# MIT-REALM/gcbf-pytorch

Hardware: NVIDIA H100
Metric: agent*steps/sec (train step, device-timed) (higher is better)
Workload: dtype f32 via 3xfp16 tensor-core products (fp32 accumulate)

## Files before the change

gcbf-pytorch_b200/csrc/gemm_wgmma_f16.cu:

```cuda
#include <cuda.h>
#include <cuda_fp16.h>
#include <stdlib.h>

#include "common.cuh"
#include "sm90_ptx.cuh"

namespace gcbf {
namespace th {

using namespace ptx;

constexpr int BM = 128;
constexpr int BK = 32;
constexpr int SUB_N = 128;
constexpr int WG_K = 16;
constexpr int NUM_THREADS = 384;
constexpr int EPI_THREADS = 256;
constexpr int KCH_MAX = 256 / BK;
constexpr int MN_BOX = 64;
constexpr int STAGES = 4;
constexpr int A_BYTES = BM * BK * 2;
constexpr int B_BYTES = SUB_N * BK * 2;
constexpr int STAGE_BYTES = 2 * A_BYTES + 2 * B_BYTES;
constexpr int PARK_PITCH = SUB_N + 8;
constexpr int PARK_BYTES = BM * PARK_PITCH * 4;
static_assert(PARK_BYTES <= STAGES * STAGE_BYTES, "the second half of a 256-wide tile is parked in the stage ring");
constexpr int SMEM_BYTES = STAGES * STAGE_BYTES + PARK_BYTES + 1024  + 256 ;

enum { EPI_FWD = 0, EPI_DGRAD = 1, EPI_WGRAD = 2 };

struct EpiParams {
  int mode;
  const float* alpha;
  const float* bias;
  int act;
  const float* relu_src;
  int ld_relu;
  const __half* relu_hi;
  int ld_relu_h;
  int accumulate;
  size_t split_stride;
  const uint32_t* amax_a; int a_sr, a_sc;
  const uint32_t* amax_b; int b_sr, b_sc;
  uint32_t* amax_out;
  __half* out_h;
  int ld_out_h;
  uint32_t* out_tile_amax;
  int out_amax_stride;
  float* colsum;
};

__host__ __device__ __forceinline__ uint32_t scale_bits_from_amax(uint32_t amax_bits) {
  const int e = (int)((amax_bits >> 23) & 0xffu);
  if (e == 0 || e == 255) return 0x3f800000u;
  int se = 127 + 14 - (e - 127);
  se = se < 2 ? 2 : (se > 252 ? 252 : se);
  return (uint32_t)se << 23;
}
__host__ __device__ __forceinline__ uint32_t inv_pow2_bits(uint32_t s_bits) { return (uint32_t)(254 - (int)(s_bits >> 23)) << 23; }

template <bool MN_MAJOR>
__device__ __forceinline__ uint64_t tile_desc(uint32_t tile_addr, int kk) {
  if (MN_MAJOR) {
    return make_smem_desc(tile_addr + (uint32_t)(kk * WG_K * 128), BK * 128, 1024, 128);
  }
  return make_smem_desc(tile_addr + (uint32_t)(kk * WG_K * 2), 16, 8 * BK * 2, BK * 2);
}

template <bool MN_MAJOR>
__device__ __forceinline__ void load_tile(uint8_t* dst, const CUtensorMap* map, uint64_t* bar, int mn0, int k0, int rows) {
  if (MN_MAJOR) {
    for (int j = 0; j < rows / MN_BOX; ++j) tma_load_2d(dst + j * (BK * 128), map, bar, mn0 + j * MN_BOX, k0);
  } else {
    tma_load_2d(dst, map, bar, k0, mn0);
  }
}

__device__ __forceinline__ void epi_sync() { asm volatile("bar.sync 1, %0;" ::"n"(EPI_THREADS) : "memory"); }

template <int BN, bool A_MN, bool B_MN>
__global__ void __launch_bounds__(NUM_THREADS, 1)
gemm_h_kernel(const __grid_constant__ CUtensorMap map_a_hi, const __grid_constant__ CUtensorMap map_a_lo,
              const __grid_constant__ CUtensorMap map_b_hi, const __grid_constant__ CUtensorMap map_b_lo,
              float* __restrict__ C, int ldc, int Mo, int No, int tiles_n, int kblocks_per_split, int kblocks_total, int KCH, EpiParams ep) {
  constexpr int NSUB = BN / SUB_N;
  constexpr int MODE = A_MN ? EPI_WGRAD : (B_MN ? EPI_DGRAD : EPI_FWD);
  extern __shared__ uint8_t smem_raw[];
  uint8_t* smem = reinterpret_cast<uint8_t*>((reinterpret_cast<uintptr_t>(smem_raw) + 1023) & ~uintptr_t(1023));
  float* park0 = reinterpret_cast<float*>(smem + STAGES * STAGE_BYTES);
  float* park1 = reinterpret_cast<float*>(smem);
  uint64_t* bars = reinterpret_cast<uint64_t*>(smem + STAGES * STAGE_BYTES + PARK_BYTES);
  uint64_t* full = bars;
  uint64_t* empty = bars + STAGES;
  uint32_t* red = reinterpret_cast<uint32_t*>(bars + 2 * STAGES);

  const int warp = threadIdx.x >> 5, lane = threadIdx.x & 31;
  const int kb0 = blockIdx.y * kblocks_per_split;
  const int kb1 = min(kblocks_total, kb0 + kblocks_per_split);
  const int nkb = kb1 - kb0;
  const int m0 = (blockIdx.x / tiles_n) * BM, n0t = (blockIdx.x % tiles_n) * BN;

  if (threadIdx.x == 0) {
    tma_prefetch_desc(&map_a_hi);
    tma_prefetch_desc(&map_a_lo);
    tma_prefetch_desc(&map_b_hi);
    tma_prefetch_desc(&map_b_lo);
    for (int s = 0; s < STAGES; ++s) { mbar_init(&full[s], 1); mbar_init(&empty[s], 2); }
    fence_barrier_init();
  }
  __syncthreads();

  if (warp < 4) {
    if (threadIdx.x == 0) {
      int stage = 0;
      uint32_t phase = 0;
      for (int sub = 0; sub < NSUB; ++sub) {
        for (int kb = kb0; kb < kb1; ++kb) {
          mbar_wait(&empty[stage], phase ^ 1);
          uint8_t* st = smem + stage * STAGE_BYTES;
          mbar_expect_tx(&full[stage], STAGE_BYTES);
          load_tile<A_MN>(st, &map_a_hi, &full[stage], m0, kb * BK, BM);
          load_tile<A_MN>(st + A_BYTES, &map_a_lo, &full[stage], m0, kb * BK, BM);
          load_tile<B_MN>(st + 2 * A_BYTES, &map_b_hi, &full[stage], n0t + sub * SUB_N, kb * BK, SUB_N);
          load_tile<B_MN>(st + 2 * A_BYTES + B_BYTES, &map_b_lo, &full[stage], n0t + sub * SUB_N, kb * BK, SUB_N);
          if (++stage == STAGES) { stage = 0; phase ^= 1; }
        }
      }
    }
  } else {
    if (nkb > 0) {
      const int tid = threadIdx.x - 128;
      const int wg = tid >> 7;
      const int wl = (tid >> 5) & 3;
      const uint32_t a_off = (uint32_t)wg * 4096u;
      int stage = 0;
      uint32_t phase = 0;
      for (int sub = 0; sub < NSUB; ++sub) {
        const int n0 = n0t + sub * SUB_N;
        float acc[64];
#pragma unroll
        for (int j = 0; j < 64; ++j) acc[j] = 0.f;
        for (int kc = 0; kc < nkb; kc += KCH) {
          const int kstart = (kb0 + kc) * BK;
          const int ia = A_MN ? (kstart >> 7) * ep.a_sr + (m0 >> 8) * ep.a_sc : (m0 >> 7) * ep.a_sr + (kstart >> 8) * ep.a_sc;
          const int ib = B_MN ? (kstart >> 7) * ep.b_sr + (n0 >> 8) * ep.b_sc : 0;
          const float cs = __uint_as_float(inv_pow2_bits(scale_bits_from_amax(__ldg(ep.amax_a + ia)))) *
                           __uint_as_float(inv_pow2_bits(scale_bits_from_amax(__ldg(ep.amax_b + ib))));
          float d[64];
#pragma unroll
          for (int j = 0; j < 64; ++j) d[j] = 0.f;
          const int kend = min(nkb, kc + KCH);
          for (int kb = kc; kb < kend; ++kb) {
            mbar_wait(&full[stage], phase);
            const uint32_t st = smem_u32(smem + stage * STAGE_BYTES);
            const uint32_t a_hi = st + a_off, a_lo = st + A_BYTES + a_off, b_hi = st + 2 * A_BYTES, b_lo = st + 2 * A_BYTES + B_BYTES;
#pragma unroll
            for (int j = 0; j < 64; ++j) fence_operand(d[j]);
            wgmma_fence();
#pragma unroll
            for (int kk = 0; kk < BK / WG_K; ++kk) {
              const uint64_t dah = tile_desc<A_MN>(a_hi, kk), dal = tile_desc<A_MN>(a_lo, kk);
              const uint64_t dbh = tile_desc<B_MN>(b_hi, kk), dbl = tile_desc<B_MN>(b_lo, kk);
              wgmma_m64n128k16_f16<A_MN ? 1 : 0, B_MN ? 1 : 0>(d, dal, dbh, (kb > kc || kk > 0) ? 1u : 0u);
              wgmma_m64n128k16_f16<A_MN ? 1 : 0, B_MN ? 1 : 0>(d, dah, dbl, 1u);
              wgmma_m64n128k16_f16<A_MN ? 1 : 0, B_MN ? 1 : 0>(d, dah, dbh, 1u);
            }
            wgmma_commit();
            wgmma_wait_all();
#pragma unroll
            for (int j = 0; j < 64; ++j) fence_operand(d[j]);
            if ((tid & 127) == 0) mbar_arrive(&empty[stage]);
            if (++stage == STAGES) { stage = 0; phase ^= 1; }
          }
#pragma unroll
          for (int j = 0; j < 64; ++j) acc[j] = __fmaf_rn(d[j], cs, acc[j]);
        }
        if (sub == 1) epi_sync();
        float* park = sub ? park1 : park0;
        const int r0 = wg * 64 + wl * 16 + (lane >> 2);
#pragma unroll
        for (int j = 0; j < 64; j += 4) {
          const int c = 8 * (j >> 2) + 2 * (lane & 3);
          *reinterpret_cast<float2*>(park + r0 * PARK_PITCH + c) = make_float2(acc[j], acc[j + 1]);
          *reinterpret_cast<float2*>(park + (r0 + 8) * PARK_PITCH + c) = make_float2(acc[j + 2], acc[j + 3]);
        }
      }
      epi_sync();

      constexpr int CG4 = BN / 4;
      constexpr int ROWS_PER_ITER = EPI_THREADS / CG4;
      const int cg = tid % CG4;
      const int c = cg * 4;
      const int col = n0t + c;
      float* const pk = (c < SUB_N ? park0 : park1) + (c & (SUB_N - 1));
      const float alpha = ep.alpha ? __ldg(ep.alpha) : 1.f;
      float bias4[4] = {0.f, 0.f, 0.f, 0.f};
      if (MODE == EPI_FWD && ep.bias) {
        const float inv_alpha = 1.f / alpha;
#pragma unroll
        for (int u = 0; u < 4; ++u) bias4[u] = (col + u < No) ? __ldg(ep.bias + col + u) * inv_alpha : 0.f;
      }
      float tmax = 0.f;
      for (int r = tid / CG4; r < BM; r += ROWS_PER_ITER) {
        const int row = m0 + r;
        float4* p = reinterpret_cast<float4*>(pk + r * PARK_PITCH);
        float v[4];
        const float4 s = *p;
        v[0] = s.x; v[1] = s.y; v[2] = s.z; v[3] = s.w;
#pragma unroll
        for (int u = 0; u < 4; ++u) {
          float y = (v[u] + bias4[u]) * alpha;
          if (MODE == EPI_FWD) {
            if (ep.act == GCBF_ACT_RELU) y = fmaxf(y, 0.f);
            else if (ep.act == GCBF_ACT_TANH) y = tanhf(y);
          }
          const bool ok = row < Mo && col + u < No;
          if (MODE == EPI_DGRAD && ok) {
            if (ep.relu_src) y = (__ldg(ep.relu_src + (size_t)row * ep.ld_relu + col + u) > 0.f) ? y : 0.f;
            else if (ep.relu_hi) y = (__half2float(ep.relu_hi[(size_t)row * ep.ld_relu_h + col + u]) > 0.f) ? y : 0.f;
          }
          v[u] = ok ? y : 0.f;
          tmax = fmaxf(tmax, fabsf(v[u]));
        }
        *p = make_float4(v[0], v[1], v[2], v[3]);
      }
      float s_tile = 1.f;
      if (MODE != EPI_WGRAD && ep.out_h) {
        const uint32_t wmax = __reduce_max_sync(0xffffffffu, __float_as_uint(tmax));
        if (lane == 0) red[tid >> 5] = wmax;
        epi_sync();
        uint32_t m = 0;
#pragma unroll
        for (int w = 0; w < EPI_THREADS / 32; ++w) m = max(m, red[w]);
        s_tile = __uint_as_float(scale_bits_from_amax(m));
        if (tid == 0 && m0 < Mo && n0t < No) ep.out_tile_amax[(size_t)(m0 >> 7) * ep.out_amax_stride + (n0t >> 8)] = m;
      }
      float out_max = 0.f;
      const bool vec_c = C && (ldc & 3) == 0 && (reinterpret_cast<uintptr_t>(C) & 15) == 0;
      const size_t plane = (size_t)Mo * ep.ld_out_h;
      for (int r = tid / CG4; r < BM; r += ROWS_PER_ITER) {
        const int row = m0 + r;
        if (row >= Mo || col >= No) continue;
        const float4 s = *reinterpret_cast<const float4*>(pk + r * PARK_PITCH);
        const float v[4] = {s.x, s.y, s.z, s.w};
        const int nv = min(4, No - col);
        if (C) {
          float* dst = C + (size_t)blockIdx.y * ep.split_stride + (size_t)row * ldc + col;
          if (ep.accumulate) {
#pragma unroll
            for (int u = 0; u < 4; ++u)
              if (u < nv) { const float o = v[u] + dst[u]; dst[u] = o; out_max = fmaxf(out_max, fabsf(o)); }
          } else if (vec_c && nv == 4) {
            *reinterpret_cast<float4*>(dst) = s;
          } else {
#pragma unroll
            for (int u = 0; u < 4; ++u)
              if (u < nv) dst[u] = v[u];
          }
        }
        if (MODE != EPI_WGRAD && ep.out_h) {
          const float y0 = v[0] * s_tile, y1 = v[1] * s_tile, y2 = v[2] * s_tile, y3 = v[3] * s_tile;
          const __half2 h01 = __floats2half2_rn(y0, y1), h23 = __floats2half2_rn(y2, y3);
          const float2 f01 = __half22float2(h01), f23 = __half22float2(h23);
          const __half2 l01 = __floats2half2_rn(__fsub_rn(y0, f01.x), __fsub_rn(y1, f01.y));
          const __half2 l23 = __floats2half2_rn(__fsub_rn(y2, f23.x), __fsub_rn(y3, f23.y));
          __half* dh = ep.out_h + (size_t)row * ep.ld_out_h + col;
          if (nv == 4) {
            *reinterpret_cast<uint2*>(dh) = make_uint2(*reinterpret_cast<const uint32_t*>(&h01), *reinterpret_cast<const uint32_t*>(&h23));
            *reinterpret_cast<uint2*>(dh + plane) = make_uint2(*reinterpret_cast<const uint32_t*>(&l01), *reinterpret_cast<const uint32_t*>(&l23));
          } else {
            const __half hs[4] = {__low2half(h01), __high2half(h01), __low2half(h23), __high2half(h23)};
            const __half ls[4] = {__low2half(l01), __high2half(l01), __low2half(l23), __high2half(l23)};
            for (int u = 0; u < nv; ++u) { dh[u] = hs[u]; dh[plane + u] = ls[u]; }
          }
        }
      }
      if (ep.amax_out && !ep.accumulate) out_max = fmaxf(out_max, tmax);
      if (MODE == EPI_DGRAD && ep.colsum) epi_sync();
      if (MODE == EPI_DGRAD && ep.colsum && tid < BN) {
        const float* pc = (tid < SUB_N ? park0 : park1) + (tid & (SUB_N - 1));
        float csum = 0.f;
#pragma unroll 8
        for (int r = 0; r < BM; ++r) csum += pc[r * PARK_PITCH];
        if (n0t + tid < No) ep.colsum[(size_t)(blockIdx.x / tiles_n) * No + n0t + tid] = csum;
      }
      if (ep.amax_out) {
        const uint32_t m = __reduce_max_sync(0xffffffffu, __float_as_uint(out_max));
        if (lane == 0 && m) atomicMax(ep.amax_out, m);
      }
    }
  }
}
__global__ void amax_kernel(const float* __restrict__ src, int ld, int rows, int cols, uint32_t* __restrict__ slot, int vec4) {
  float m = 0.f;
  if (vec4) {
    const int w = cols >> 2;
    for (int r = blockIdx.x; r < rows; r += gridDim.x) {
      const float4* p = reinterpret_cast<const float4*>(src + (size_t)r * ld);
      for (int c = threadIdx.x; c < w; c += blockDim.x) {
        const float4 x = __ldg(p + c);
        m = fmaxf(fmaxf(m, fmaxf(fabsf(x.x), fabsf(x.y))), fmaxf(fabsf(x.z), fabsf(x.w)));
      }
    }
  } else {
    for (int r = blockIdx.x; r < rows; r += gridDim.x)
      for (int c = threadIdx.x; c < cols; c += blockDim.x) m = fmaxf(m, fabsf(__ldg(src + (size_t)r * ld + c)));
  }
  const uint32_t w = __reduce_max_sync(0xffffffffu, __float_as_uint(m));
  __shared__ uint32_t part[32];
  if ((threadIdx.x & 31) == 0) part[threadIdx.x >> 5] = w;
  __syncthreads();
  if (threadIdx.x < 32) {
    uint32_t v = threadIdx.x < (blockDim.x >> 5) ? part[threadIdx.x] : 0u;
    v = __reduce_max_sync(0xffffffffu, v);
    if (threadIdx.x == 0 && v) atomicMax(slot, v);
  }
}

constexpr int SPLIT_ROWS = 64;
__global__ void split_h_kernel(const float* __restrict__ src, int ld, int rows, int cols, const uint32_t* __restrict__ amax,
                               __half* __restrict__ dst, int ld_h, float* __restrict__ colsum) {
  const float s = __uint_as_float(scale_bits_from_amax(__ldg(amax)));
  const int c = (blockIdx.x * 32 + threadIdx.x) * 2;
  const int r0 = blockIdx.y * SPLIT_ROWS;
  const size_t plane = (size_t)rows * ld_h;
  float s0 = 0.f, s1 = 0.f;
  if (c < cols) {
    const bool pair = (c + 1 < cols);
    const int r1 = min(rows, r0 + SPLIT_ROWS);
    for (int r = r0 + threadIdx.y; r < r1; r += blockDim.y) {
      const float* p = src + (size_t)r * ld + c;
      const float x0 = __ldg(p), x1 = pair ? __ldg(p + 1) : 0.f;
      const float y0 = x0 * s, y1 = x1 * s;
      const __half2 hi = __floats2half2_rn(y0, y1);
      const float2 hf = __half22float2(hi);
      const __half2 lo = __floats2half2_rn(__fsub_rn(y0, hf.x), __fsub_rn(y1, hf.y));
      __half* d = dst + (size_t)r * ld_h + c;
      if (pair) {
        *reinterpret_cast<__half2*>(d) = hi;
        *reinterpret_cast<__half2*>(d + plane) = lo;
      } else {
        d[0] = __low2half(hi);
        d[plane] = __low2half(lo);
      }
      s0 += x0; s1 += x1;
    }
  }
  if (colsum) {
    __shared__ float red[8][64];
    red[threadIdx.y][2 * threadIdx.x] = s0;
    red[threadIdx.y][2 * threadIdx.x + 1] = s1;
    __syncthreads();
    if (threadIdx.y == 0) {
      float t0 = 0.f, t1 = 0.f;
#pragma unroll
      for (int y = 0; y < 8; ++y) { t0 += red[y][2 * threadIdx.x]; t1 += red[y][2 * threadIdx.x + 1]; }
      if (c < cols) colsum[(size_t)blockIdx.y * cols + c] = t0;
      if (c + 1 < cols) colsum[(size_t)blockIdx.y * cols + c + 1] = t1;
    }
  }
}

__device__ __forceinline__ void split4(const float4 x, float s, uint2& hi, uint2& lo) {
  const float y0 = x.x * s, y1 = x.y * s, y2 = x.z * s, y3 = x.w * s;
  const __half2 h01 = __floats2half2_rn(y0, y1), h23 = __floats2half2_rn(y2, y3);
  const float2 f01 = __half22float2(h01), f23 = __half22float2(h23);
  const __half2 l01 = __floats2half2_rn(__fsub_rn(y0, f01.x), __fsub_rn(y1, f01.y));
  const __half2 l23 = __floats2half2_rn(__fsub_rn(y2, f23.x), __fsub_rn(y3, f23.y));
  hi.x = *reinterpret_cast<const uint32_t*>(&h01); hi.y = *reinterpret_cast<const uint32_t*>(&h23);
  lo.x = *reinterpret_cast<const uint32_t*>(&l01); lo.y = *reinterpret_cast<const uint32_t*>(&l23);
}

__global__ void __launch_bounds__(256) split_h4_kernel(const float* __restrict__ src, int ld, int rows, int cols,
                                                       const uint32_t* __restrict__ amax, __half* __restrict__ dst, int ld_h,
                                                       float* __restrict__ colsum) {
  const float s = __uint_as_float(scale_bits_from_amax(__ldg(amax)));
  const int c = (blockIdx.x * 32 + threadIdx.x) * 4;
  const int r0 = blockIdx.y * SPLIT_ROWS;
  const size_t plane = (size_t)rows * ld_h;
  float cs[4] = {0.f, 0.f, 0.f, 0.f};
  if (c < cols) {
    const int r1 = min(rows, r0 + SPLIT_ROWS);
    for (int r = r0 + threadIdx.y; r < r1; r += 32) {
      float4 x[4];
#pragma unroll
      for (int u = 0; u < 4; ++u)
        x[u] = (r + 8 * u < r1) ? __ldg(reinterpret_cast<const float4*>(src + (size_t)(r + 8 * u) * ld + c)) : make_float4(0.f, 0.f, 0.f, 0.f);
#pragma unroll
      for (int u = 0; u < 4; ++u) {
        if (r + 8 * u < r1) {
          uint2 hi, lo;
          split4(x[u], s, hi, lo);
          __half* d = dst + (size_t)(r + 8 * u) * ld_h + c;
          *reinterpret_cast<uint2*>(d) = hi;
          *reinterpret_cast<uint2*>(d + plane) = lo;
          cs[0] += x[u].x; cs[1] += x[u].y; cs[2] += x[u].z; cs[3] += x[u].w;
        }
      }
    }
  }
  if (colsum) {
    __shared__ float red[8][128];
#pragma unroll
    for (int j = 0; j < 4; ++j) red[threadIdx.y][4 * threadIdx.x + j] = cs[j];
    __syncthreads();
    if (threadIdx.y < 4) {
      const int col = threadIdx.y * 32 + threadIdx.x;
      float t = 0.f;
#pragma unroll
      for (int y = 0; y < 8; ++y) t += red[y][col];
      const int gc = blockIdx.x * 128 + col;
      if (gc < cols) colsum[(size_t)blockIdx.y * cols + gc] = t;
    }
  }
}

constexpr int kSplitMaxBatch = 16;
struct SplitBatch {
  const float* src[kSplitMaxBatch];
  uint32_t* amax[kSplitMaxBatch];
  __half* dst[kSplitMaxBatch];
  int ld[kSplitMaxBatch], rows[kSplitMaxBatch], cols[kSplitMaxBatch], ld_h[kSplitMaxBatch];
};

__global__ void __launch_bounds__(256) amax_batched_kernel(const __grid_constant__ SplitBatch b) {
  const int t = blockIdx.z;
  const int ld = b.ld[t], rows = b.rows[t], cols = b.cols[t];
  const int warp = threadIdx.x >> 5, lane = threadIdx.x & 31;
  const float* __restrict__ src = b.src[t];
  const bool vec = ((cols & 3) == 0 && (ld & 3) == 0 && (reinterpret_cast<uintptr_t>(src) & 15) == 0);
  float m = 0.f;
  for (int r = blockIdx.x * 8 + warp; r < rows; r += gridDim.x * 8) {
    const float* row = src + (size_t)r * ld;
    if (vec) {
      const float4* p = reinterpret_cast<const float4*>(row);
      for (int c = lane; c < (cols >> 2); c += 32) {
        const float4 x = __ldg(p + c);
        m = fmaxf(fmaxf(m, fmaxf(fabsf(x.x), fabsf(x.y))), fmaxf(fabsf(x.z), fabsf(x.w)));
      }
    } else {
      for (int c = lane; c < cols; c += 32) m = fmaxf(m, fabsf(__ldg(row + c)));
    }
  }
  const uint32_t w = __reduce_max_sync(0xffffffffu, __float_as_uint(m));
  __shared__ uint32_t part[8];
  if (lane == 0) part[warp] = w;
  __syncthreads();
  if (threadIdx.x < 32) {
    uint32_t v = threadIdx.x < 8 ? part[threadIdx.x] : 0u;
    v = __reduce_max_sync(0xffffffffu, v);
    if (threadIdx.x == 0 && v) atomicMax(b.amax[t], v);
  }
}

__global__ void __launch_bounds__(256) split_batched_kernel(const __grid_constant__ SplitBatch b) {
  const int t = blockIdx.z;
  const int ld = b.ld[t], rows = b.rows[t], cols = b.cols[t], ld_h = b.ld_h[t];
  const int c = (blockIdx.x * 32 + threadIdx.x) * 2;
  const int r0 = blockIdx.y * SPLIT_ROWS;
  if (c >= cols || r0 >= rows) return;
  const float* __restrict__ src = b.src[t];
  __half* __restrict__ dst = b.dst[t];
  const float s = __uint_as_float(scale_bits_from_amax(*b.amax[t]));
  const size_t plane = (size_t)rows * ld_h;
  const bool pair = (c + 1 < cols);
  const int r1 = min(rows, r0 + SPLIT_ROWS);
  for (int r = r0 + threadIdx.y; r < r1; r += blockDim.y) {
    const float* p = src + (size_t)r * ld + c;
    const float y0 = __ldg(p) * s, y1 = pair ? __ldg(p + 1) * s : 0.f;
    const __half2 hi = __floats2half2_rn(y0, y1);
    const float2 hf = __half22float2(hi);
    const __half2 lo = __floats2half2_rn(__fsub_rn(y0, hf.x), __fsub_rn(y1, hf.y));
    __half* d = dst + (size_t)r * ld_h + c;
    if (pair) {
      *reinterpret_cast<__half2*>(d) = hi;
      *reinterpret_cast<__half2*>(d + plane) = lo;
    } else {
      d[0] = __low2half(hi);
      d[plane] = __low2half(lo);
    }
  }
}

typedef CUresult (*EncodeTiledFn)(CUtensorMap*, CUtensorMapDataType, cuuint32_t, void*, const cuuint64_t*, const cuuint64_t*,
                                  const cuuint32_t*, const cuuint32_t*, CUtensorMapInterleave, CUtensorMapSwizzle,
                                  CUtensorMapL2promotion, CUtensorMapFloatOOBfill);

static EncodeTiledFn get_encode_fn() {
  static EncodeTiledFn fn = nullptr;
  if (!fn) {
    void* p = nullptr;
    cudaDriverEntryPointQueryResult q;
    if (cudaGetDriverEntryPoint("cuTensorMapEncodeTiled", &p, cudaEnableDefault, &q) == cudaSuccess && p) fn = (EncodeTiledFn)p;
  }
  return fn;
}

static int make_map(CUtensorMap* map, const __half* base, int rows, int cols, int ld_h, bool mn_major, int tile_rows) {
  EncodeTiledFn fn = get_encode_fn();
  if (!fn) { set_error("cuTensorMapEncodeTiled entry point unavailable"); return GCBF_E_CUDA; }
  cuuint64_t dims[2] = {(cuuint64_t)cols, (cuuint64_t)rows};
  cuuint64_t strides[1] = {(cuuint64_t)ld_h * 2};
  cuuint32_t box[2] = {(cuuint32_t)(mn_major ? MN_BOX : BK), (cuuint32_t)(mn_major ? BK : tile_rows)};
  cuuint32_t estr[2] = {1, 1};
  CUresult r = fn(map, CU_TENSOR_MAP_DATA_TYPE_FLOAT16, 2, const_cast<__half*>(base), dims, strides, box, estr,
                  CU_TENSOR_MAP_INTERLEAVE_NONE, mn_major ? CU_TENSOR_MAP_SWIZZLE_128B : CU_TENSOR_MAP_SWIZZLE_64B,
                  CU_TENSOR_MAP_L2_PROMOTION_L2_256B, CU_TENSOR_MAP_FLOAT_OOB_FILL_NONE);
  if (r != CUDA_SUCCESS) {
    set_error("cuTensorMapEncodeTiled failed (%d) rows=%d cols=%d ld=%d mn=%d", (int)r, rows, cols, ld_h, (int)mn_major);
    return GCBF_E_CUDA;
  }
  return GCBF_OK;
}

static bool g_env_read = false;
static int g_kch = 4;
static int g_kch_dgrad = 8;

struct Operand {
  const __half* hi; int rows; int cols; int ld_h; bool mn_major;
  const __half* lo() const { return hi + (size_t)rows * ld_h; }
};
struct OutH {
  __half* hi; int rows; int cols; int ld_h; uint32_t* tile_amax; int amax_stride;
};

template <int BN, bool A_MN, bool B_MN>
static int launch(const Operand& A, const Operand& B, float* C, int ldc, int Mo, int No, int Kc, int splits, EpiParams ep,
                  const OutH* oh, cudaStream_t st) {
  if (!g_env_read) {
    const char* kc = getenv("GCBF_TC_KCH");
    if (kc && atoi(kc) >= 1 && atoi(kc) <= KCH_MAX) g_kch = atoi(kc);
    const char* kd = getenv("GCBF_TC_KCH_DGRAD");
    if (kd && atoi(kd) >= 1 && atoi(kd) <= KCH_MAX) g_kch_dgrad = atoi(kd);
    if (kc && !kd) g_kch_dgrad = g_kch > 4 ? g_kch : g_kch_dgrad;
    g_env_read = true;
  }
  if ((ep.a_sr || ep.a_sc || ep.b_sr || ep.b_sc) && g_kch > 4) { set_error("tile-scaled operands need promotion chunks of <= 128 K-elements (GCBF_TC_KCH <= 4)"); return GCBF_E_UNSUPPORTED; }
  if constexpr (BN != 256 || A_MN) {
    if (oh || ep.colsum) { set_error("companion emission / column sums need a 256-wide forward or data-grad launch"); return GCBF_E_UNSUPPORTED; }
  }
  CUtensorMap mah, mal, mbh, mbl;
  if (int rc = make_map(&mah, A.hi, A.rows, A.cols, A.ld_h, A_MN, BM)) return rc;
  if (int rc = make_map(&mal, A.lo(), A.rows, A.cols, A.ld_h, A_MN, BM)) return rc;
  if (int rc = make_map(&mbh, B.hi, B.rows, B.cols, B.ld_h, B_MN, SUB_N)) return rc;
  if (int rc = make_map(&mbl, B.lo(), B.rows, B.cols, B.ld_h, B_MN, SUB_N)) return rc;
  if (oh) {
    ep.out_h = oh->hi; ep.ld_out_h = oh->ld_h; ep.out_tile_amax = oh->tile_amax; ep.out_amax_stride = oh->amax_stride;
  }
  static bool attr_set = false;
  if (!attr_set) {
    GCBF_CUDA_OK(cudaFuncSetAttribute(gemm_h_kernel<BN, A_MN, B_MN>, cudaFuncAttributeMaxDynamicSharedMemorySize, SMEM_BYTES));
    attr_set = true;
  }
  const int tiles_m = ceil_div(Mo, BM), tiles_n = ceil_div(No, BN);
  const int kblocks = ceil_div(Kc, BK);
  const int kch = (!A_MN && B_MN && !(ep.b_sr || ep.b_sc)) ? g_kch_dgrad : g_kch;
  const int kps = ceil_div(ceil_div(kblocks, splits), kch) * kch;
  const int nsplit = ceil_div(kblocks, kps);
  float* part = nullptr;
  float* colsum_part = nullptr;
  float* const colsum = ep.colsum;
  const int accumulate = ep.accumulate;
  if (nsplit > 1) {
    GCBF_CUDA_OK(scratch_alloc((void**)&part, (size_t)nsplit * Mo * No * 4, st));
    ep.split_stride = (size_t)Mo * No;
    ep.accumulate = 0;
  }
  if (colsum) {
    GCBF_CUDA_OK(scratch_alloc((void**)&colsum_part, (size_t)tiles_m * No * 4, st));
    ep.colsum = colsum_part;
  }
  gemm_h_kernel<BN, A_MN, B_MN><<<dim3(tiles_m * tiles_n, nsplit), NUM_THREADS, SMEM_BYTES, st>>>(mah, mal, mbh, mbl, part ? part : C,
                                                                                                 part ? No : ldc, Mo, No, tiles_n, kps,
                                                                                                 kblocks, kch, ep);
  GCBF_LAUNCH_OK();
  if (part) {
    GCBF_CUDA_OK(add_partials(part, nsplit, Mo, No, C, ldc, accumulate, st));
    GCBF_CUDA_OK(scratch_free(part, st));
  }
  if (colsum_part) {
    GCBF_CUDA_OK(add_partials(colsum_part, tiles_m, 1, No, colsum, No, 1, st));
    GCBF_CUDA_OK(scratch_free(colsum_part, st));
  }
  return GCBF_OK;
}

static int check_plane(const void* p, int ld_h, const char* what) {
  if (!p || (reinterpret_cast<uintptr_t>(p) & 15) || (ld_h & 7)) {
    set_error("%s: fp16 companion must be 16-byte aligned with a pitch that is a multiple of 8 halves (ptr=%p ld=%d)", what, p, ld_h);
    return GCBF_E_INVALID;
  }
  return GCBF_OK;
}

}
}

using namespace gcbf;

extern "C" int gcbf_amax_f32(const float* src, int ld, int rows, int cols, void* amax_slot, int accumulate, void* stream) {
  GCBF_REQUIRE(amax_slot && rows >= 0 && cols >= 0 && ld >= cols, "gcbf_amax_f32: bad arguments rows=%d cols=%d ld=%d", rows, cols, ld);
  cudaStream_t st = as_stream(stream);
  if (!accumulate) GCBF_CUDA_OK(cudaMemsetAsync(amax_slot, 0, 4, st));
  if (rows == 0 || cols == 0) return GCBF_OK;
  GCBF_REQUIRE(src, "gcbf_amax_f32: null src");
  const int vec4 = ((cols & 3) == 0 && (ld & 3) == 0 && (reinterpret_cast<uintptr_t>(src) & 15) == 0) ? 1 : 0;
  const int work = vec4 ? cols / 4 : cols;
  const int threads = work >= 256 ? 256 : (work >= 128 ? 128 : 64);
  const int blocks = (int)imin64(rows, (int64_t)kNumSMs * (2048 / threads));
  th::amax_kernel<<<blocks, threads, 0, st>>>(src, ld, rows, cols, reinterpret_cast<uint32_t*>(amax_slot), vec4);
  GCBF_LAUNCH_OK();
  return GCBF_OK;
}

extern "C" int gcbf_split_f16(const float* src, int ld, int rows, int cols, const void* amax_slot, void* dst, int ld_h,
                              float* colsum, int colsum_accumulate, void* stream) {
  GCBF_REQUIRE(amax_slot && dst && rows >= 0 && cols >= 0 && ld >= cols && ld_h >= cols, "gcbf_split_f16: bad arguments rows=%d cols=%d", rows, cols);
  if (int rc = th::check_plane(dst, ld_h, "gcbf_split_f16")) return rc;
  cudaStream_t st = as_stream(stream);
  if (colsum && !colsum_accumulate) GCBF_CUDA_OK(cudaMemsetAsync(colsum, 0, (size_t)cols * 4, st));
  if (rows == 0 || cols == 0) return GCBF_OK;
  GCBF_REQUIRE(src, "gcbf_split_f16: null src");
  dim3 block(32, 8);
  const int strips = ceil_div(rows, th::SPLIT_ROWS);
  float* part = nullptr;
  if (colsum) GCBF_CUDA_OK(scratch_alloc((void**)&part, (size_t)strips * cols * 4, st));
  if ((cols & 3) == 0 && (ld & 3) == 0 && (reinterpret_cast<uintptr_t>(src) & 15) == 0) {
    dim3 grid(ceil_div(cols, 128), strips);
    th::split_h4_kernel<<<grid, block, 0, st>>>(src, ld, rows, cols, reinterpret_cast<const uint32_t*>(amax_slot),
                                               reinterpret_cast<__half*>(dst), ld_h, part);
  } else {
    dim3 grid(ceil_div(cols, 64), strips);
    th::split_h_kernel<<<grid, block, 0, st>>>(src, ld, rows, cols, reinterpret_cast<const uint32_t*>(amax_slot),
                                              reinterpret_cast<__half*>(dst), ld_h, part);
  }
  GCBF_LAUNCH_OK();
  if (part) {
    GCBF_CUDA_OK(add_partials(part, strips, 1, cols, colsum, cols, 1, st));
    GCBF_CUDA_OK(scratch_free(part, st));
  }
  return GCBF_OK;
}

extern "C" int gcbf_amax_split_batched(const gcbf_split_desc* descs, int count, void* stream) {
  GCBF_REQUIRE(descs && count >= 0, "gcbf_amax_split_batched: bad arguments");
  cudaStream_t st = as_stream(stream);
  for (int base = 0; base < count; base += th::kSplitMaxBatch) {
    const int nb = min(th::kSplitMaxBatch, count - base);
    th::SplitBatch b{};
    int max_rows = 0, max_cols = 0;
    for (int i = 0; i < nb; ++i) {
      const gcbf_split_desc& d = descs[base + i];
      GCBF_REQUIRE(d.src && d.amax_slot && d.dst && d.rows > 0 && d.cols > 0 && d.ld >= d.cols && d.ld_h >= d.cols,
                   "gcbf_amax_split_batched: descriptor %d", base + i);
      if (int rc = th::check_plane(d.dst, d.ld_h, "gcbf_amax_split_batched")) return rc;
      b.src[i] = d.src; b.amax[i] = reinterpret_cast<uint32_t*>(d.amax_slot); b.dst[i] = reinterpret_cast<__half*>(d.dst);
      b.ld[i] = d.ld; b.rows[i] = d.rows; b.cols[i] = d.cols; b.ld_h[i] = d.ld_h;
      max_rows = max(max_rows, d.rows); max_cols = max(max_cols, d.cols);
      GCBF_CUDA_OK(cudaMemsetAsync(d.amax_slot, 0, 4, st));
    }
    th::amax_batched_kernel<<<dim3(min(ceil_div(max_rows, 8), 8 * kNumSMs), 1, nb), 256, 0, st>>>(b);
    GCBF_LAUNCH_OK();
    th::split_batched_kernel<<<dim3(ceil_div(max_cols, 64), ceil_div(max_rows, th::SPLIT_ROWS), nb), dim3(32, 8), 0, st>>>(b);
    GCBF_LAUNCH_OK();
  }
  return GCBF_OK;
}

extern "C" int gcbf_linear_h_supported(int M, int N, int K) {
  return (M >= 256 && N >= 96 && K >= 96 && (long long)M * N * K >= (1ll << 24)) ? 1 : 0;
}

static int check_h16(const gcbf_h16* h, const char* what, int rows, int cols) {
  if (!h || !h->buf || !h->amax || h->rows != rows || h->cols != cols || h->ld < cols) {
    set_error("%s: companion descriptor (expected [%d x %d])", what, rows, cols);
    return GCBF_E_INVALID;
  }
  return th::check_plane(h->buf, h->ld, what);
}

extern "C" int gcbf_linear_fwd_t(const gcbf_h16* X, const gcbf_h16* W, const float* bias, const float* inv_sigma, int act, float* Y, int ldy,
                                 const gcbf_h16* Yh, void* out_amax, int M, int N, int K, void* stream) {
  GCBF_REQUIRE(M > 0 && N > 0 && K > 0 && (Y || Yh) && (!Y || ldy >= N), "gcbf_linear_fwd_t: bad arguments M=%d N=%d K=%d", M, N, K);
  if (int rc = check_h16(X, "gcbf_linear_fwd_t X", M, K)) return rc;
  if (int rc = check_h16(W, "gcbf_linear_fwd_t W", N, K)) return rc;
  GCBF_REQUIRE(W->amax_row_stride == 0 && W->amax_col_stride == 0, "gcbf_linear_fwd_t: the weight companion must be per-tensor scaled");
  cudaStream_t st = as_stream(stream);
  th::EpiParams ep{};
  ep.mode = th::EPI_FWD; ep.alpha = inv_sigma; ep.bias = bias; ep.act = act;
  ep.amax_a = reinterpret_cast<const uint32_t*>(X->amax); ep.a_sr = X->amax_row_stride; ep.a_sc = X->amax_col_stride;
  ep.amax_b = reinterpret_cast<const uint32_t*>(W->amax);
  ep.amax_out = reinterpret_cast<uint32_t*>(out_amax);
  if (out_amax) GCBF_CUDA_OK(cudaMemsetAsync(out_amax, 0, 4, st));
  th::OutH oh{};
  if (Yh) {
    if (int rc = check_h16(Yh, "gcbf_linear_fwd_t Yh", M, N)) return rc;
    GCBF_REQUIRE(N > 128 && Yh->amax_row_stride == ceil_div(N, 256) && Yh->amax_col_stride == 1, "gcbf_linear_fwd_t: emitted companions are tile-scaled (N > 128, amax strides (ceil(N/256), 1))");
    oh = th::OutH{reinterpret_cast<__half*>(Yh->buf), M, N, Yh->ld, reinterpret_cast<uint32_t*>(Yh->amax), Yh->amax_row_stride};
  }
  th::Operand A{reinterpret_cast<const __half*>(X->buf), M, K, X->ld, false}, B{reinterpret_cast<const __half*>(W->buf), N, K, W->ld, false};
  return (N > 128) ? th::launch<256, false, false>(A, B, Y, ldy, M, N, K, 1, ep, Yh ? &oh : nullptr, st)
                   : th::launch<128, false, false>(A, B, Y, ldy, M, N, K, 1, ep, nullptr, st);
}

extern "C" int gcbf_linear_bwd_data_t(const gcbf_h16* dZ, const gcbf_h16* W, const float* inv_sigma, const float* relu_src, int ld_relu,
                                      const gcbf_h16* relu_h, float* dX, int lddx, int accumulate, const gcbf_h16* dXh, float* colsum,
                                      void* out_amax, int M, int N, int K, void* stream) {
  GCBF_REQUIRE(M > 0 && N > 0 && K > 0 && (dX || dXh) && (!dX || lddx >= K), "gcbf_linear_bwd_data_t: bad arguments M=%d N=%d K=%d", M, N, K);
  GCBF_REQUIRE(!relu_src || ld_relu >= K, "gcbf_linear_bwd_data_t: ld_relu");
  GCBF_REQUIRE(!(relu_src && relu_h) && !(accumulate && (dXh || colsum)), "gcbf_linear_bwd_data_t: conflicting options");
  if (int rc = check_h16(dZ, "gcbf_linear_bwd_data_t dZ", M, N)) return rc;
  if (int rc = check_h16(W, "gcbf_linear_bwd_data_t W", N, K)) return rc;
  GCBF_REQUIRE(W->amax_row_stride == 0 && W->amax_col_stride == 0, "gcbf_linear_bwd_data_t: the weight companion must be per-tensor scaled");
  if (relu_h) { if (int rc = check_h16(relu_h, "gcbf_linear_bwd_data_t relu_h", M, K)) return rc; }
  cudaStream_t st = as_stream(stream);
  th::EpiParams ep{};
  ep.mode = th::EPI_DGRAD; ep.alpha = inv_sigma; ep.relu_src = relu_src; ep.ld_relu = ld_relu; ep.accumulate = accumulate;
  if (relu_h) { ep.relu_hi = reinterpret_cast<const __half*>(relu_h->buf); ep.ld_relu_h = relu_h->ld; }
  ep.amax_a = reinterpret_cast<const uint32_t*>(dZ->amax); ep.a_sr = dZ->amax_row_stride; ep.a_sc = dZ->amax_col_stride;
  ep.amax_b = reinterpret_cast<const uint32_t*>(W->amax);
  ep.amax_out = reinterpret_cast<uint32_t*>(out_amax);
  ep.colsum = colsum;
  if (out_amax) GCBF_CUDA_OK(cudaMemsetAsync(out_amax, 0, 4, st));
  th::OutH oh{};
  if (dXh) {
    if (int rc = check_h16(dXh, "gcbf_linear_bwd_data_t dXh", M, K)) return rc;
    GCBF_REQUIRE(K > 128 && dXh->amax_row_stride == ceil_div(K, 256) && dXh->amax_col_stride == 1, "gcbf_linear_bwd_data_t: emitted companions are tile-scaled (K > 128, amax strides (ceil(K/256), 1))");
    oh = th::OutH{reinterpret_cast<__half*>(dXh->buf), M, K, dXh->ld, reinterpret_cast<uint32_t*>(dXh->amax), dXh->amax_row_stride};
  }
  th::Operand A{reinterpret_cast<const __half*>(dZ->buf), M, N, dZ->ld, false}, B{reinterpret_cast<const __half*>(W->buf), N, K, W->ld, true};
  return (K > 128) ? th::launch<256, false, true>(A, B, dX, lddx, M, K, N, 1, ep, dXh ? &oh : nullptr, st)
                   : th::launch<128, false, true>(A, B, dX, lddx, M, K, N, 1, ep, nullptr, st);
}

extern "C" int gcbf_linear_bwd_weight_t(const gcbf_h16* dZ, const gcbf_h16* X, const float* inv_sigma, float* dW, int lddw, int accumulate,
                                        int M, int N, int K, void* stream) {
  GCBF_REQUIRE(M > 0 && N > 0 && K > 0 && lddw >= K && dW, "gcbf_linear_bwd_weight_t: bad arguments M=%d N=%d K=%d", M, N, K);
  if (int rc = check_h16(dZ, "gcbf_linear_bwd_weight_t dZ", M, N)) return rc;
  if (int rc = check_h16(X, "gcbf_linear_bwd_weight_t X", M, K)) return rc;
  cudaStream_t st = as_stream(stream);
  th::EpiParams ep{};
  ep.mode = th::EPI_WGRAD; ep.alpha = inv_sigma; ep.accumulate = accumulate;
  ep.amax_a = reinterpret_cast<const uint32_t*>(dZ->amax); ep.a_sr = dZ->amax_row_stride; ep.a_sc = dZ->amax_col_stride;
  ep.amax_b = reinterpret_cast<const uint32_t*>(X->amax); ep.b_sr = X->amax_row_stride; ep.b_sc = X->amax_col_stride;
  const int BN = (K > 128) ? 256 : 128;
  const int tiles = ceil_div(N, th::BM) * ceil_div(K, BN);
  int splits = 1;
  if (tiles < kNumSMs) splits = max(1, min(ceil_div(M, 256), kNumSMs / tiles));
  th::Operand A{reinterpret_cast<const __half*>(dZ->buf), M, N, dZ->ld, true}, B{reinterpret_cast<const __half*>(X->buf), M, K, X->ld, true};
  return (BN == 256) ? th::launch<256, true, true>(A, B, dW, lddw, N, K, M, splits, ep, nullptr, st)
                     : th::launch<128, true, true>(A, B, dW, lddw, N, K, M, splits, ep, nullptr, st);
}

static gcbf_h16 per_tensor(const void* buf, int ld, const void* amax, int rows, int cols) {
  gcbf_h16 h;
  h.buf = const_cast<void*>(buf); h.amax = const_cast<void*>(amax); h.ld = ld; h.rows = rows; h.cols = cols; h.amax_row_stride = 0; h.amax_col_stride = 0;
  return h;
}

extern "C" int gcbf_linear_fwd_h(const void* Xh, int ldxh, const void* x_amax, const void* Wh, int ldwh, const void* w_amax,
                                 const float* bias, const float* inv_sigma, float* Y, int ldy, int M, int N, int K, int act,
                                 void* out_amax, void* stream) {
  GCBF_REQUIRE(Y && x_amax && w_amax, "gcbf_linear_fwd_h: null pointer");
  const gcbf_h16 X = per_tensor(Xh, ldxh, x_amax, M, K), W = per_tensor(Wh, ldwh, w_amax, N, K);
  return gcbf_linear_fwd_t(&X, &W, bias, inv_sigma, act, Y, ldy, nullptr, out_amax, M, N, K, stream);
}

extern "C" int gcbf_linear_bwd_data_h(const void* dZh, int lddzh, const void* dz_amax, const void* Wh, int ldwh,
                                      const void* w_amax, const float* inv_sigma, const float* relu_src, int ld_relu, float* dX,
                                      int lddx, int M, int N, int K, int accumulate, void* out_amax, void* stream) {
  GCBF_REQUIRE(dX && dz_amax && w_amax, "gcbf_linear_bwd_data_h: null pointer");
  const gcbf_h16 dZ = per_tensor(dZh, lddzh, dz_amax, M, N), W = per_tensor(Wh, ldwh, w_amax, N, K);
  return gcbf_linear_bwd_data_t(&dZ, &W, inv_sigma, relu_src, ld_relu, nullptr, dX, lddx, accumulate, nullptr, nullptr, out_amax, M, N, K, stream);
}

extern "C" int gcbf_linear_bwd_weight_h(const void* dZh, int lddzh, const void* dz_amax, const void* Xh, int ldxh,
                                        const void* x_amax, const float* inv_sigma, float* dW, int lddw, int M, int N, int K,
                                        int accumulate, void* stream) {
  GCBF_REQUIRE(dW && dz_amax && x_amax, "gcbf_linear_bwd_weight_h: null pointer");
  const gcbf_h16 dZ = per_tensor(dZh, lddzh, dz_amax, M, N), X = per_tensor(Xh, ldxh, x_amax, M, K);
  return gcbf_linear_bwd_weight_t(&dZ, &X, inv_sigma, dW, lddw, accumulate, M, N, K, stream);
}
```

gcbf-pytorch_b200/csrc/sm90_ptx.cuh:

```cuda
#pragma once
#include <cuda.h>
#include <stdint.h>

namespace gcbf {
namespace ptx {

__device__ __forceinline__ uint32_t smem_u32(const void* p) { return (uint32_t)__cvta_generic_to_shared(p); }

__device__ __forceinline__ void mbar_init(uint64_t* bar, uint32_t count) {
  asm volatile("mbarrier.init.shared::cta.b64 [%0], %1;" ::"r"(smem_u32(bar)), "r"(count));
}
__device__ __forceinline__ void mbar_expect_tx(uint64_t* bar, uint32_t bytes) {
  asm volatile("mbarrier.arrive.expect_tx.shared::cta.b64 _, [%0], %1;" ::"r"(smem_u32(bar)), "r"(bytes) : "memory");
}
__device__ __forceinline__ void mbar_arrive(uint64_t* bar) {
  asm volatile("mbarrier.arrive.shared::cta.b64 _, [%0];" ::"r"(smem_u32(bar)) : "memory");
}
__device__ __forceinline__ uint32_t mbar_try_wait(uint64_t* bar, uint32_t parity) {
  uint32_t ok;
  asm volatile(
      "{\n\t"
      ".reg .pred p;\n\t"
      "mbarrier.try_wait.parity.shared::cta.b64 p, [%1], %2;\n\t"
      "selp.u32 %0, 1, 0, p;\n\t"
      "}"
      : "=r"(ok)
      : "r"(smem_u32(bar)), "r"(parity)
      : "memory");
  return ok;
}
__device__ __forceinline__ void mbar_wait(uint64_t* bar, uint32_t parity) {
  while (!mbar_try_wait(bar, parity)) {
  }
}
__device__ __forceinline__ void fence_barrier_init() { asm volatile("fence.mbarrier_init.release.cluster;" ::: "memory"); }

__device__ __forceinline__ void tma_load_2d(void* smem_dst, const CUtensorMap* map, uint64_t* bar, int c0, int c1) {
  asm volatile(
      "cp.async.bulk.tensor.2d.shared::cluster.global.mbarrier::complete_tx::bytes [%0], [%1, {%3, %4}], [%2];" ::"r"(
          smem_u32(smem_dst)),
      "l"(reinterpret_cast<uint64_t>(map)), "r"(smem_u32(bar)), "r"(c0), "r"(c1)
      : "memory");
}
__device__ __forceinline__ void tma_prefetch_desc(const CUtensorMap* map) {
  asm volatile("prefetch.tensormap [%0];" ::"l"(reinterpret_cast<uint64_t>(map)) : "memory");
}

__device__ __forceinline__ void wgmma_fence() { asm volatile("wgmma.fence.sync.aligned;" ::: "memory"); }
__device__ __forceinline__ void wgmma_commit() { asm volatile("wgmma.commit_group.sync.aligned;" ::: "memory"); }
__device__ __forceinline__ void wgmma_wait_all() { asm volatile("wgmma.wait_group.sync.aligned 0;" ::: "memory"); }
__device__ __forceinline__ void fence_operand(float& r) { asm volatile("" : "+f"(r)::"memory"); }

template <int TA, int TB>
__device__ __forceinline__ void wgmma_m64n128k16_f16(float (&d)[64], uint64_t desc_a, uint64_t desc_b, uint32_t scale_d) {
  asm volatile(
      "{\n\t"
      ".reg .pred p;\n\t"
      "setp.ne.b32 p, %66, 0;\n\t"
      "wgmma.mma_async.sync.aligned.m64n128k16.f32.f16.f16 "
      "{%0, %1, %2, %3, %4, %5, %6, %7, %8, %9, %10, %11, %12, %13, %14, %15, "
      "%16, %17, %18, %19, %20, %21, %22, %23, %24, %25, %26, %27, %28, %29, %30, %31, "
      "%32, %33, %34, %35, %36, %37, %38, %39, %40, %41, %42, %43, %44, %45, %46, %47, "
      "%48, %49, %50, %51, %52, %53, %54, %55, %56, %57, %58, %59, %60, %61, %62, %63}, "
      "%64, %65, p, 1, 1, %67, %68;\n\t"
      "}\n"
      : "+f"(d[0]), "+f"(d[1]), "+f"(d[2]), "+f"(d[3]), "+f"(d[4]), "+f"(d[5]), "+f"(d[6]), "+f"(d[7]), "+f"(d[8]), "+f"(d[9]),
        "+f"(d[10]), "+f"(d[11]), "+f"(d[12]), "+f"(d[13]), "+f"(d[14]), "+f"(d[15]), "+f"(d[16]), "+f"(d[17]), "+f"(d[18]),
        "+f"(d[19]), "+f"(d[20]), "+f"(d[21]), "+f"(d[22]), "+f"(d[23]), "+f"(d[24]), "+f"(d[25]), "+f"(d[26]), "+f"(d[27]),
        "+f"(d[28]), "+f"(d[29]), "+f"(d[30]), "+f"(d[31]), "+f"(d[32]), "+f"(d[33]), "+f"(d[34]), "+f"(d[35]), "+f"(d[36]),
        "+f"(d[37]), "+f"(d[38]), "+f"(d[39]), "+f"(d[40]), "+f"(d[41]), "+f"(d[42]), "+f"(d[43]), "+f"(d[44]), "+f"(d[45]),
        "+f"(d[46]), "+f"(d[47]), "+f"(d[48]), "+f"(d[49]), "+f"(d[50]), "+f"(d[51]), "+f"(d[52]), "+f"(d[53]), "+f"(d[54]),
        "+f"(d[55]), "+f"(d[56]), "+f"(d[57]), "+f"(d[58]), "+f"(d[59]), "+f"(d[60]), "+f"(d[61]), "+f"(d[62]), "+f"(d[63])
      : "l"(desc_a), "l"(desc_b), "r"(scale_d), "n"(TA), "n"(TB)
      : "memory");
}

__device__ __forceinline__ uint64_t make_smem_desc(uint32_t smem_addr, uint32_t lbo_bytes, uint32_t sbo_bytes, int swizzle_bytes) {
  uint64_t d = 0;
  d |= (uint64_t)((smem_addr >> 4) & 0x3FFF);
  d |= (uint64_t)((lbo_bytes >> 4) & 0x3FFF) << 16;
  d |= (uint64_t)((sbo_bytes >> 4) & 0x3FFF) << 32;
  d |= (uint64_t)(swizzle_bytes == 128 ? 1 : swizzle_bytes == 64 ? 2 : swizzle_bytes == 32 ? 3 : 0) << 62;
  return d;
}

}
}
```

Before: 343,800.

## Double-buffer WGMMA accumulators and rebalance registers between producer and consumers

Consumer warpgroups now alternate between two accumulator register sets, so each chunk's wgmma group stays in flight (wait<1>) while the previous chunk's scaled promotion into acc runs. Smem stages are released one step late to match. The producer warpgroup gives up registers via setmaxnreg.dec and the consumers take more via setmaxnreg.inc, to hold the extra 64-float buffer without spilling. This is meant to hide the wgmma drain and FMA promotion latency, at the cost of more register pressure and more complex chunk/sub-tile bookkeeping.

Result: faster. 356,100, median of 6 (+3.6%).

```diff
diff --git a/gcbf-pytorch_b200/csrc/gemm_wgmma_f16.cu b/gcbf-pytorch_b200/csrc/gemm_wgmma_f16.cu
--- a/gcbf-pytorch_b200/csrc/gemm_wgmma_f16.cu
+++ b/gcbf-pytorch_b200/csrc/gemm_wgmma_f16.cu
@@ -111,6 +111,7 @@
   __syncthreads();
 
   if (warp < 4) {
+    setmaxnreg_dec<40>();
     if (threadIdx.x == 0) {
       int stage = 0;
       uint32_t phase = 0;
@@ -128,55 +129,25 @@
       }
     }
   } else {
+    setmaxnreg_inc<232>();
     if (nkb > 0) {
       const int tid = threadIdx.x - 128;
       const int wg = tid >> 7;
       const int wl = (tid >> 5) & 3;
+      const bool leader = (tid & 127) == 0;
       const uint32_t a_off = (uint32_t)wg * 4096u;
+      const int nch = (nkb + KCH - 1) / KCH;
+      int nchunks = NSUB * nch;
+      asm("" : "+r"(nchunks));
       int stage = 0;
       uint32_t phase = 0;
-      for (int sub = 0; sub < NSUB; ++sub) {
-        const int n0 = n0t + sub * SUB_N;
-        float acc[64];
-#pragma unroll
-        for (int j = 0; j < 64; ++j) acc[j] = 0.f;
-        for (int kc = 0; kc < nkb; kc += KCH) {
-          const int kstart = (kb0 + kc) * BK;
-          const int ia = A_MN ? (kstart >> 7) * ep.a_sr + (m0 >> 8) * ep.a_sc : (m0 >> 7) * ep.a_sr + (kstart >> 8) * ep.a_sc;
-          const int ib = B_MN ? (kstart >> 7) * ep.b_sr + (n0 >> 8) * ep.b_sc : 0;
-          const float cs = __uint_as_float(inv_pow2_bits(scale_bits_from_amax(__ldg(ep.amax_a + ia)))) *
-                           __uint_as_float(inv_pow2_bits(scale_bits_from_amax(__ldg(ep.amax_b + ib))));
-          float d[64];
-#pragma unroll
-          for (int j = 0; j < 64; ++j) d[j] = 0.f;
-          const int kend = min(nkb, kc + KCH);
-          for (int kb = kc; kb < kend; ++kb) {
-            mbar_wait(&full[stage], phase);
-            const uint32_t st = smem_u32(smem + stage * STAGE_BYTES);
-            const uint32_t a_hi = st + a_off, a_lo = st + A_BYTES + a_off, b_hi = st + 2 * A_BYTES, b_lo = st + 2 * A_BYTES + B_BYTES;
-#pragma unroll
-            for (int j = 0; j < 64; ++j) fence_operand(d[j]);
-            wgmma_fence();
-#pragma unroll
-            for (int kk = 0; kk < BK / WG_K; ++kk) {
-              const uint64_t dah = tile_desc<A_MN>(a_hi, kk), dal = tile_desc<A_MN>(a_lo, kk);
-              const uint64_t dbh = tile_desc<B_MN>(b_hi, kk), dbl = tile_desc<B_MN>(b_lo, kk);
-              wgmma_m64n128k16_f16<A_MN ? 1 : 0, B_MN ? 1 : 0>(d, dal, dbh, (kb > kc || kk > 0) ? 1u : 0u);
-              wgmma_m64n128k16_f16<A_MN ? 1 : 0, B_MN ? 1 : 0>(d, dah, dbl, 1u);
-              wgmma_m64n128k16_f16<A_MN ? 1 : 0, B_MN ? 1 : 0>(d, dah, dbh, 1u);
-            }
-            wgmma_commit();
-            wgmma_wait_all();
-#pragma unroll
-            for (int j = 0; j < 64; ++j) fence_operand(d[j]);
-            if ((tid & 127) == 0) mbar_arrive(&empty[stage]);
-            if (++stage == STAGES) { stage = 0; phase ^= 1; }
-          }
-#pragma unroll
-          for (int j = 0; j < 64; ++j) acc[j] = __fmaf_rn(d[j], cs, acc[j]);
-        }
-        if (sub == 1) epi_sync();
-        float* park = sub ? park1 : park0;
+      int held = -1;
+      float cs_prev = 0.f;
+      float acc[64], d0[64], d1[64];
+#pragma unroll
+      for (int j = 0; j < 64; ++j) acc[j] = 0.f;
+
+      auto park_acc = [&](float* park) {
         const int r0 = wg * 64 + wl * 16 + (lane >> 2);
 #pragma unroll
         for (int j = 0; j < 64; j += 4) {
@@ -184,6 +155,66 @@
           *reinterpret_cast<float2*>(park + r0 * PARK_PITCH + c) = make_float2(acc[j], acc[j + 1]);
           *reinterpret_cast<float2*>(park + (r0 + 8) * PARK_PITCH + c) = make_float2(acc[j + 2], acc[j + 3]);
         }
+      };
+      auto promote = [&](float (&p)[64], float cs) {
+#pragma unroll
+        for (int j = 0; j < 64; ++j) fence_operand(p[j]);
+#pragma unroll
+        for (int j = 0; j < 64; ++j) acc[j] = __fmaf_rn(p[j], cs, acc[j]);
+      };
+      auto run_chunk = [&](float (&d)[64], float (&p)[64], int g) {
+        const int sub = (NSUB > 1 && g >= nch) ? 1 : 0;
+        const int kc = (g - sub * nch) * KCH;
+        const int n0 = n0t + sub * SUB_N;
+        const int kstart = (kb0 + kc) * BK;
+        const int ia = A_MN ? (kstart >> 7) * ep.a_sr + (m0 >> 8) * ep.a_sc : (m0 >> 7) * ep.a_sr + (kstart >> 8) * ep.a_sc;
+        const int ib = B_MN ? (kstart >> 7) * ep.b_sr + (n0 >> 8) * ep.b_sc : 0;
+        const float cs = __uint_as_float(inv_pow2_bits(scale_bits_from_amax(__ldg(ep.amax_a + ia)))) *
+                         __uint_as_float(inv_pow2_bits(scale_bits_from_amax(__ldg(ep.amax_b + ib))));
+        const int kend = min(nkb, kc + KCH);
+        for (int kb = kc; kb < kend; ++kb) {
+          mbar_wait(&full[stage], phase);
+          const uint32_t st = smem_u32(smem + stage * STAGE_BYTES);
+          const uint32_t a_hi = st + a_off, a_lo = st + A_BYTES + a_off, b_hi = st + 2 * A_BYTES, b_lo = st + 2 * A_BYTES + B_BYTES;
+#pragma unroll
+          for (int j = 0; j < 64; ++j) fence_operand(d[j]);
+          wgmma_fence();
+#pragma unroll
+          for (int kk = 0; kk < BK / WG_K; ++kk) {
+            const uint64_t dah = tile_desc<A_MN>(a_hi, kk), dal = tile_desc<A_MN>(a_lo, kk);
+            const uint64_t dbh = tile_desc<B_MN>(b_hi, kk), dbl = tile_desc<B_MN>(b_lo, kk);
+            wgmma_m64n128k16_f16<A_MN ? 1 : 0, B_MN ? 1 : 0>(d, dal, dbh, (kb > kc || kk > 0) ? 1u : 0u);
+            wgmma_m64n128k16_f16<A_MN ? 1 : 0, B_MN ? 1 : 0>(d, dah, dbl, 1u);
+            wgmma_m64n128k16_f16<A_MN ? 1 : 0, B_MN ? 1 : 0>(d, dah, dbh, 1u);
+          }
+          wgmma_commit();
+          wgmma_wait<1>();
+          if (held >= 0 && leader) mbar_arrive(&empty[held]);
+          held = stage;
+          if (++stage == STAGES) { stage = 0; phase ^= 1; }
+          if (kb == kc && g > 0) {
+            promote(p, cs_prev);
+            if (NSUB > 1 && g == nch) {
+              park_acc(park0);
+#pragma unroll
+              for (int j = 0; j < 64; ++j) acc[j] = 0.f;
+            }
+          }
+        }
+        cs_prev = cs;
+      };
+      auto finish = [&](float (&d)[64]) {
+        wgmma_wait<0>();
+        if (leader) mbar_arrive(&empty[held]);
+        promote(d, cs_prev);
+        if (NSUB > 1) epi_sync();
+        park_acc(NSUB > 1 ? park1 : park0);
+      };
+      for (int g = 0;; g += 2) {
+        run_chunk(d0, d1, g);
+        if (g + 1 == nchunks) { finish(d0); break; }
+        run_chunk(d1, d0, g + 1);
+        if (g + 2 == nchunks) { finish(d1); break; }
       }
       epi_sync();
 
diff --git a/gcbf-pytorch_b200/csrc/sm90_ptx.cuh b/gcbf-pytorch_b200/csrc/sm90_ptx.cuh
--- a/gcbf-pytorch_b200/csrc/sm90_ptx.cuh
+++ b/gcbf-pytorch_b200/csrc/sm90_ptx.cuh
@@ -48,8 +48,14 @@
 
 __device__ __forceinline__ void wgmma_fence() { asm volatile("wgmma.fence.sync.aligned;" ::: "memory"); }
 __device__ __forceinline__ void wgmma_commit() { asm volatile("wgmma.commit_group.sync.aligned;" ::: "memory"); }
-__device__ __forceinline__ void wgmma_wait_all() { asm volatile("wgmma.wait_group.sync.aligned 0;" ::: "memory"); }
+template <int N>
+__device__ __forceinline__ void wgmma_wait() { asm volatile("wgmma.wait_group.sync.aligned %0;" ::"n"(N) : "memory"); }
 __device__ __forceinline__ void fence_operand(float& r) { asm volatile("" : "+f"(r)::"memory"); }
+
+template <int R>
+__device__ __forceinline__ void setmaxnreg_dec() { asm volatile("setmaxnreg.dec.sync.aligned.u32 %0;" ::"n"(R)); }
+template <int R>
+__device__ __forceinline__ void setmaxnreg_inc() { asm volatile("setmaxnreg.inc.sync.aligned.u32 %0;" ::"n"(R)); }
 
 template <int TA, int TB>
 __device__ __forceinline__ void wgmma_m64n128k16_f16(float (&d)[64], uint64_t desc_a, uint64_t desc_b, uint32_t scale_d) {
```
